# ToughStoneX/Self-Supervised-MVS

Measured on AMD Instinct MI355X. Metric: depth-samples/sec (N=3, 640x512, D=192), higher is better.
Workload: dtype f32

## Files before the change

### self-supervised-mvs_amd/_lib.py

```python
from __future__ import annotations

import contextlib
import ctypes as C
import os

_HERE = os.path.dirname(os.path.abspath(__file__))
LIB_PATH = os.path.join(_HERE, "libmvs_hip.so")

_f = C.c_void_p
_i = C.c_int
_ll = C.c_longlong
_s = C.c_void_p
_fl = C.c_float

class MvsUnetBlock(C.Structure):
    _fields_ = [("transposed", _i), ("stride", _i), ("src", _i), ("skip", _i), ("eps", _fl), ("momentum", _fl),
                ("cin", _i), ("cout", _i), ("d", _i), ("h", _i), ("w", _i)]


class MvsFeatBlock(C.Structure):
    _fields_ = [("cin", _i), ("cout", _i), ("ks", _i), ("stride", _i), ("eps", _fl), ("momentum", _fl), ("w_channels_last", _i),
                ("h", _i), ("w", _i)]


# ... 170 lines not shown
        msg = self._mvs_last_error().decode("utf-8", "replace")
        if rc in (-1, -2, -4):
            raise ValueError("%s failed (%d): %s" % (name, rc, msg))
        raise RuntimeError("%s failed (%d): %s" % (name, rc, msg))

    def raw(self, name: str, *args):
        return getattr(self, "_" + name)(*args)

    def launch_trace(self):
        buf = C.create_string_buffer(4096)
        self._mvs_launch_trace(buf, len(buf))
        return [s for s in buf.value.decode().split(",") if s]

    def get_tuning(self, key: str) -> int:
        v = _i()
        self.call("mvs_get_tuning", key.encode(), C.byref(v))
        return v.value

    @contextlib.contextmanager
    def tuning(self, **knobs):
        old = []
        try:
            for key, val in knobs.items():
                old.append((key, self.get_tuning(key)))
                self.call("mvs_set_tuning", key.encode(), int(val))
            yield self
        finally:
            for key, val in reversed(old):
                self.call("mvs_set_tuning", key.encode(), val)


_INSTANCE = None

DEFAULT_TUNING = {"k8": 7, "xcd": 1, "side_pre": 1, "conv_pers": 1, "conv_pers_min": 1024, "conv_pers_nw": 8, "wgrad_pers": 1, "conv_small": 1, "tr2pw": 1, "sweep_bwd": 0, "wgrad_small": 0, "wgrad_groups": 768, "wgrad8_groups": 192, "wgrad8_gs": 2, "wgrad8_nch": 2, "cout1_h4": 1, "wgrad2d_batch": 2048, "sweep_fwd": 3}


def get() -> MvsLib:
    global _INSTANCE
    if _INSTANCE is None:
        _INSTANCE = MvsLib()
        for item in filter(None, os.environ.get("MVS_TUNING", "").split(",")):
            key, _, val = item.partition("=")
            DEFAULT_TUNING[key.strip()] = int(val)
            _INSTANCE.call("mvs_set_tuning", key.strip().encode(), int(val))
    return _INSTANCE


class KernelTimer:

    def __init__(self, only=None, names=None):
        self.only = only
        self.names = names
        self.events = {}

    def wants(self, name, tag):
        return self.only is None or name in self.only or tag in self.only

    def add(self, name, tag, ev0, ev1):
        self.events.setdefault((name, tag), []).append((ev0, ev1))

    _REG_NAMES = frozenset(("mvs_conv3d_fwd", "mvs_convT3d_fwd", "mvs_conv3d_dgrad", "mvs_convT3d_dgrad", "mvs_conv3d_wgrad", "mvs_convT3d_wgrad",
                            "mvs_bn_relu_fwd_slots", "mvs_bn_relu_bwd_slots", "mvs_bn_bwd_reduce_slots", "mvs_conv3d_pack_weights_batch"))

    def allows_c_entry(self, lib, blocks):
        if self.names is None:
            return False
        hit = self.names & self._REG_NAMES
# ... 57 lines not shown
```

### self-supervised-mvs_amd/csrc/conv3d.hip

```cpp
#include "mvs_rt.h"
#include "conv_map.h"

#include "conv_args.h"

__device__ __forceinline__ void conv_pack_weights_item(const float* __restrict__ w, float* __restrict__ wp, int geom, int CC,
                                                       int Cin, int Cout, int NB, int layout, int flip, int idx) {
    const int j = idx & 3, lane = (idx >> 2) & 63;
    const int nb = (idx >> 8) % NB, kk = (idx >> 8) / NB;
    const int co = nb * 16 + (lane & 15);
    int ks, chunk = 0, cls = 0;
    if (geom == GEOM_TR2_PW) {
        int k0 = 0;
        for (cls = 0; cls < 4; ++cls) {
            int n = tr2p_ntaps(cls) * CC / 16;
            if (kk < k0 + n) break;
            k0 += n;
        }
        ks = kk - k0;
        const int kf = 16 * ks + 4 * (lane >> 4) + j;
        const int tp = kf / CC, cip = kf % CC, n = lane & 15, pw = n >> 3, cop = n & 7;
        int dd, dh, dw, kd, kh;
        tr2p_tap(cls, tp, dd, dh, dw, kd, kh);
        int kw = tr2p_kw(pw, dw);
        float v = 0.f;
// ... 64 lines not shown
template <int NIT, class Map>
__device__ __forceinline__ void stage_load(float4 (&v)[NIT], int (&off)[NIT], int tid, int nitems, Map map) {
#pragma unroll
    for (int k = 0; k < NIT; ++k) {
        const int i = tid + 256 * k;
        off[k] = -1;
        v[k] = make_float4(0.f, 0.f, 0.f, 0.f);
        if (i < nitems) {
            const float* src = nullptr;
            map(i, src, off[k]);
            if (src) v[k] = *reinterpret_cast<const float4*>(src);
        }
    }
}
template <int NIT>
__device__ __forceinline__ void stage_store(float* __restrict__ lds, const float4 (&v)[NIT], const int (&off)[NIT]) {
#pragma unroll
    for (int k = 0; k < NIT; ++k)
        if (off[k] >= 0) *reinterpret_cast<float4*>(lds + off[k]) = v[k];
}
template <int NITEMS, class Map>
__device__ __forceinline__ void stage_batched(float* __restrict__ lds, int tid, Map map) {
    constexpr int NIT = (NITEMS + 255) / 256;
    constexpr int BATCH = NIT < 12 ? NIT : 12;
#pragma unroll
    for (int k0 = 0; k0 < NIT; k0 += BATCH) {
        float4 v[BATCH];
        int off[BATCH];
        stage_load<BATCH>(v, off, tid, NITEMS - 256 * k0, [&](int i, const float*& src, int& o) { map(i + 256 * k0, src, o); });
        stage_store<BATCH>(lds, v, off);
    }
}

template <int GEOM, int CC, int NB, int SIDE>
__global__ __launch_bounds__(256) void conv_igemm_kernel(ConvArgs a) {
    using G = ConvGeom<GEOM>;
    constexpr int CCP = CC + 4;
    constexpr int NR = G::RD * G::RH * G::RW;
    constexpr int MB = G::MB;
    constexpr int CQ = CC / 4;
    __shared__ __attribute__((aligned(16))) float tile[NR * CCP];
    __shared__ int tapoff[32];
    __shared__ float red[4 * NB * 16 * 2];

    const int tid = threadIdx.x, lane = tid & 63, wave = tid >> 6;
    const int g = lane >> 4, l15 = lane & 15;
    const int nb0 = blockIdx.y * NB;

    int t = blockIdx.x;
    const int tw = t % a.ntw; t /= a.ntw;
    const int th = t % a.nth; t /= a.nth;
    const int td = t % a.ntd; t /= a.ntd;
    const int b = t;
    const int qd0 = td * G::TQD, qh0 = th * G::TQH, qw0 = tw * G::TQW;

    if (tid < 32) {
        int off = 0;
        if (G::PW) {
            if (tid < 18) {
                int cls = 0, k0 = 0;
                for (; cls < 4; ++cls) {
                    int n = tr2p_ntaps(cls);
                    if (tid < k0 + n) break;
                    k0 += n;
                }
                int dd, dh, dw, kd, kh;
                tr2p_tap(cls, tid - k0, dd, dh, dw, kd, kh);
                off = ((dd * G::RH + dh) * G::RW + dw) * CCP;
            }
        } else if (G::BASE == GEOM_TR2) {
            if (tid < 27) {
                int cls = 0, k0 = 0;
                for (; cls < 8; ++cls) {
                    int n = tr2_ntaps(cls);
                    if (tid < k0 + n) break;
                    k0 += n;
                }
                int dd, dh, dw, kd, kh, kw;
                tr2_tap(cls, tid - k0, dd, dh, dw, kd, kh, kw);
                off = ((dd * G::RH + dh) * G::RW + dw) * CCP;
            }
        } else if (tid < 27) {
            off = (((tid / 9) * G::RH + (tid / 3) % 3) * G::RW + tid % 3) * CCP;
        }
        tapoff[tid] = off;
    }

    int baseA[MB];
#pragma unroll
    for (int mb = 0; mb < MB; ++mb) {
        const int f = wave * MB + mb;
        const int qd_l = f / G::TQH, qh_l = f % G::TQH;
        baseA[mb] = (((qd_l * G::IS) * G::RH + qh_l * G::IS) * G::RW + l15 * G::IS) * CCP;
    }

    f32x4 acc[MB][NB];
    float st1[NB], st2[NB];
    float bmu[NB], bis[NB], bsc[NB], bsh[NB];
#pragma unroll
    for (int nb = 0; nb < NB; ++nb) {
        st1[nb] = 0.f; st2[nb] = 0.f;
        bmu[nb] = bis[nb] = bsc[nb] = bsh[nb] = 0.f;
        if (SIDE && a.bn_raw) {
            const int co = G::PW ? (l15 & 7) : (nb0 + nb) * 16 + l15;
            if (co < a.Cout) { bmu[nb] = a.bn_stats[co]; bis[nb] = a.bn_stats[a.Cout + co]; bsc[nb] = a.bn_stats[2 * a.Cout + co]; bsh[nb] = a.bn_stats[3 * a.Cout + co]; }
        }
    }

    const int nchunks = G::BASE == GEOM_TR2 ? 1 : a.Cin / CC;
    const int KSF = ksteps_for(27, CC);

    constexpr int EG = (MB * NB * 8 <= 64) ? MB : 1;
    constexpr bool SIDE_PRE = SIDE == 2 && NB == 1 && EG == MB;
    auto pd_of = [&](int cls) { return G::PW ? (cls >> 1) & 1 : (cls >> 2) & 1; };
    auto ph_of = [&](int cls) { return G::PW ? cls & 1 : (cls >> 1) & 1; };
    auto pw_of = [&](int cls) { return G::PW ? (l15 >> 3) : cls & 1; };
    auto load_side = [&](int cls, int mb0, float (&sk)[EG][4][NB], float (&rwv)[EG][4][NB]) {
#pragma unroll
        for (int e = 0; e < EG; ++e) {
            const int f = wave * MB + mb0 + e;
            const int qd = qd0 + f / G::TQH, qh = qh0 + f % G::TQH;
            const int od = qd * G::OS + pd_of(cls), oh = qh * G::OS + ph_of(cls);
#pragma unroll
            for (int r = 0; r < 4; ++r) {
                const int qw = qw0 + 4 * g + r;
                const int ow = qw * G::OS + pw_of(cls);
                const size_t obase = ((((size_t)b * a.Do + od) * a.Ho + oh) * a.Wo + ow) * a.Cout;
#pragma unroll
                for (int nb = 0; nb < NB; ++nb) {
                    const int co = G::PW ? (l15 & 7) : (nb0 + nb) * 16 + l15;
                    const bool ok = qd < a.QD && qh < a.QH && qw < a.QW && co < a.Cout;
                    sk[e][r][nb] = (ok && a.skip) ? a.skip[obase + co] : 0.f;
                    rwv[e][r][nb] = (ok && a.bn_raw) ? a.bn_raw[obase + co] : 0.f;
                }
            }
        }
    };
    float skp[SIDE_PRE ? MB : 1][4][NB], rwp[SIDE_PRE ? MB : 1][4][NB];

    for (int cls = 0; cls < G::NCLS; ++cls) {
#pragma unroll
        for (int mb = 0; mb < MB; ++mb)
#pragma unroll
            for (int nb = 0; nb < NB; ++nb) acc[mb][nb] = (f32x4){0.f, 0.f, 0.f, 0.f};
        if constexpr (SIDE_PRE) {
            if (a.skip || a.bn_raw) load_side(cls, 0, skp, rwp);
        }

        for (int chunk = 0; chunk < nchunks; ++chunk) {
            if (cls == 0) {
                __syncthreads();
                stage_batched<NR * CQ>(tile, tid, [&](int i, const float*& src, int& o) {
                    const int vox = i / CQ, cq = i % CQ;
                    const int rw = vox % G::RW, rh = (vox / G::RW) % G::RH, rd = vox / (G::RW * G::RH);
                    const int id = qd0 * G::IS + rd - G::PAD, ih = qh0 * G::IS + rh - G::PAD,
                              iw = qw0 * G::IS + rw - G::PAD;
                    o = vox * CCP + 4 * cq;
                    if (id >= 0 && id < a.Di && ih >= 0 && ih < a.Hi && iw >= 0 && iw < a.Wi)
                        src = a.x + ((((size_t)b * a.Di + id) * a.Hi + ih) * a.Wi + iw) * a.Cin + chunk * CC + 4 * cq;
                });
                __syncthreads();
            }
            int KS, kk0, tapbase;
            if (G::PW) {
                KS = tr2p_ntaps(cls) * CC / 16;
                tapbase = tr2p_tap_prefix(cls);
                kk0 = tapbase * CC / 16;
            } else if (G::BASE == GEOM_TR2) {
                KS = tr2_ntaps(cls) * CC / 16;
                tapbase = tr2_tap_prefix(cls);
                kk0 = tapbase * CC / 16;
            } else {
                KS = KSF;
                tapbase = 0;
                kk0 = chunk * KSF;
            }
            constexpr int PD = G::BASE == GEOM_TR2 ? 1 : (NB == 1 ? 4 : 2);
            float4 bq[PD][NB], af[MB];
            auto load_b = [&](int ks, float4 (&dst)[NB]) {
                const int kc = ks < KS ? ks : KS - 1;
#pragma unroll
                for (int nb = 0; nb < NB; ++nb)
                    dst[nb] = *reinterpret_cast<const float4*>(a.wp + (((size_t)(kk0 + kc) * a.nb_total + nb0 + nb) * 64 + lane) * 4);
            };
            auto load_a = [&](int ks, float4 (&dst)[MB]) {
                const int kc = ks < KS ? ks : KS - 1;
                const int kflat = 16 * kc + 4 * g;
                const int aoff = tapoff[tapbase + kflat / CC] + kflat % CC;
#pragma unroll
                for (int mb = 0; mb < MB; ++mb) dst[mb] = *reinterpret_cast<const float4*>(&tile[baseA[mb] + aoff]);
            };
#pragma unroll
            for (int u = 0; u < PD; ++u) load_b(u, bq[u]);
            load_a(0, af);
            for (int ks0 = 0; ks0 < KS; ks0 += PD) {
#pragma unroll
                for (int u = 0; u < PD; ++u) {
                    const int ks = ks0 + u;
                    if (ks < KS) {
                        float4 an[MB];
                        load_a(ks + 1, an);
#pragma unroll
                        for (int mb = 0; mb < MB; ++mb)
#pragma unroll
                            for (int nb = 0; nb < NB; ++nb) {
                                acc[mb][nb] = MVS_MFMA_16x16x4(af[mb].x, bq[u][nb].x, acc[mb][nb]);
                                acc[mb][nb] = MVS_MFMA_16x16x4(af[mb].y, bq[u][nb].y, acc[mb][nb]);
                                acc[mb][nb] = MVS_MFMA_16x16x4(af[mb].z, bq[u][nb].z, acc[mb][nb]);
                                acc[mb][nb] = MVS_MFMA_16x16x4(af[mb].w, bq[u][nb].w, acc[mb][nb]);
                            }
                        load_b(ks + PD, bq[u]);
#pragma unroll
                        for (int mb = 0; mb < MB; ++mb) af[mb] = an[mb];
                    }
                }
            }
        }

#pragma unroll
        for (int mb0 = 0; mb0 < MB; mb0 += EG) {
            float sk[EG][4][NB], rwv[EG][4][NB];
            if (SIDE && !SIDE_PRE && (a.skip || a.bn_raw)) load_side(cls, mb0, sk, rwv);
#pragma unroll
            for (int e = 0; e < EG; ++e) {
                const int mb = mb0 + e;
                const int f = wave * MB + mb;
                const int qd = qd0 + f / G::TQH, qh = qh0 + f % G::TQH;
                if (qd >= a.QD || qh >= a.QH) continue;
                const int od = qd * G::OS + pd_of(cls), oh = qh * G::OS + ph_of(cls);
#pragma unroll
                for (int r = 0; r < 4; ++r) {
                    const int qw = qw0 + 4 * g + r;
                    if (qw >= a.QW) continue;
                    const int ow = qw * G::OS + pw_of(cls);
                    const size_t obase = ((((size_t)b * a.Do + od) * a.Ho + oh) * a.Wo + ow) * a.Cout;
#pragma unroll
                    for (int nb = 0; nb < NB; ++nb) {
                        const int co = G::PW ? (l15 & 7) : (nb0 + nb) * 16 + l15;
                        if (co >= a.Cout) continue;
                        float v = acc[mb][nb][r];
                        float sv1 = v, sv2 = v * v;
                        if (a.scale) v = v * a.scale[co] + a.shift[co];
                        else if (a.shift) v = v + a.shift[co];
                        if (a.relu) v = fmaxf(v, 0.f);
                        if (SIDE && a.skip) v += SIDE_PRE ? skp[SIDE_PRE ? mb : 0][r][nb] : sk[e][r][nb];
                        if (SIDE && a.bn_raw) {
                            const float rw = SIDE_PRE ? rwp[SIDE_PRE ? mb : 0][r][nb] : rwv[e][r][nb];
                            sv1 = (rw * bsc[nb] + bsh[nb] > 0.f) ? v : 0.f;
                            sv2 = sv1 * ((rw - bmu[nb]) * bis[nb]);
                        }
                        st1[nb] += sv1;
                        st2[nb] += sv2;
                        a.y[obase + co] = v;
                    }
                }
            }
        }
    }

    if (a.slots) {
#pragma unroll
        for (int nb = 0; nb < NB; ++nb) {
            float s1 = st1[nb], s2 = st2[nb];
            s1 += __shfl_xor(s1, 16); s1 += __shfl_xor(s1, 32);
            s2 += __shfl_xor(s2, 16); s2 += __shfl_xor(s2, 32);
            if (G::PW) { s1 += __shfl_xor(s1, 8); s2 += __shfl_xor(s2, 8); }
            if (lane < 16) {
                red[((wave * NB + nb) * 16 + lane) * 2 + 0] = s1;
// ... 919 lines not shown
    }
    red[slice][el] = (s0 + s1) + (s2 + s3);
    __syncthreads();
    if (slice == 0 && e < n) {
        float t = 0.f;
#pragma unroll
        for (int k = 0; k < 16; ++k) t += red[k][el];
        const int cg = e % CG, cx = (e / CG) % CX, tap = e / (CG * CX);
        gw[((size_t)cg * CX + cx) * 27 + tap] = t;
    }
}

static int pick_cc(int geom, int cin) {
    if (geom == GEOM_TR2) return cin;
    if (geom == GEOM_S2) return 8;
    return (cin % 16 == 0) ? 16 : 8;
}

static int pick_cc_k(int geom, int kgeom, int cin) {
    if (g_tune.cc_wide) {
        if (kgeom == GEOM_S1_SMALL && (cin == 32 || cin == 64)) return cin;
        if (kgeom == GEOM_S2_SMALL && (cin == 16 || cin == 32)) return cin;
    }
    return pick_cc(geom, cin);
}

static size_t packed_floats(int geom, int cin, int cout) {
    const int cc = pick_cc(geom, cin);
    int nb = mvs_cdiv(cout, 16);
    if (nb == 3) nb = 4;
    return (size_t)total_ksteps(geom, cin, cc) * nb * 256;
}

template <int GEOM>
static const char* igemm_label() {
    return GEOM == GEOM_S1 ? "conv_igemm s1" : GEOM == GEOM_S2 ? "conv_igemm s2" : GEOM == GEOM_TR2 ? "conv_igemm tr2" :
           GEOM == GEOM_S1_SMALL ? "conv_igemm s1_small" : GEOM == GEOM_S2_SMALL ? "conv_igemm s2_small" :
           GEOM == GEOM_TR2_SMALL ? "conv_igemm tr2_small" : GEOM == GEOM_TR2_PW ? "conv_igemm tr2_pw" : "conv_igemm";
}

template <int GEOM, int CC>
static int launch_igemm_nb(const ConvArgs& a, int NB, int nblocks, hipStream_t st) {
    dim3 grid(nblocks, a.nb_total / NB), block(256);
    if (a.skip || a.bn_raw) {
        switch (NB) {
            case 1:
                if (g_tune.side_pre) MVS_LAUNCH((conv_igemm_kernel<GEOM, CC, 1, 2>), grid, block, 0, st, a);
                else MVS_LAUNCH((conv_igemm_kernel<GEOM, CC, 1, 1>), grid, block, 0, st, a);
                break;
            case 2: MVS_LAUNCH((conv_igemm_kernel<GEOM, CC, 2, 1>), grid, block, 0, st, a); break;
            case 4: MVS_LAUNCH((conv_igemm_kernel<GEOM, CC, 4, 1>), grid, block, 0, st, a); break;
            default: mvs_set_error("conv igemm: Cout tile count %d unsupported", NB); return MVS_ERR_UNSUPPORTED;
        }
        return mvs_check_launch(igemm_label<GEOM>());
    }
    switch (NB) {
        case 1: MVS_LAUNCH((conv_igemm_kernel<GEOM, CC, 1, 0>), grid, block, 0, st, a); break;
        case 2: MVS_LAUNCH((conv_igemm_kernel<GEOM, CC, 2, 0>), grid, block, 0, st, a); break;
        case 4: MVS_LAUNCH((conv_igemm_kernel<GEOM, CC, 4, 0>), grid, block, 0, st, a); break;
        default: mvs_set_error("conv igemm: Cout tile count %d unsupported", NB); return MVS_ERR_UNSUPPORTED;
    }
    return mvs_check_launch(igemm_label<GEOM>());
}

static void igemm_tiling(int geom, int B, int QD, int QH, int QW, int cout, int& kgeom, int& NB, int& nblocks) {
    const int nb_total = mvs_cdiv(cout, 16) == 3 ? 4 : mvs_cdiv(cout, 16);
    nblocks = B * mvs_cdiv(QD, geom_tqd(geom)) * mvs_cdiv(QH, geom_tqh(geom)) * mvs_cdiv(QW, 16);
    NB = nb_total;
    if (g_tune.conv_split && nblocks < 512 && NB > 1) NB = 1;
    kgeom = geom;
    const long thr = (long)g_tune.conv_small_wgs * (geom == GEOM_S2 ? 24 : (geom == GEOM_S1 ? 3 : 1));
    if (g_tune.conv_small == 2 || (g_tune.conv_small == 1 && (long)nblocks * (nb_total / NB) < thr)) {
        kgeom = geom + GEOM_S1_SMALL;
        nblocks = B * mvs_cdiv(QD, geom_tqd(kgeom)) * mvs_cdiv(QH, geom_tqh(kgeom)) * mvs_cdiv(QW, 16);
    }
}

struct Epilogue {
    const float* scale; const float* shift; const float* skip; int relu;
    double* slots; int nslots;
    const float* bn_raw; const float* bn_stats;
};

struct IgemmPlan {
    int geom, wlayout, flip, B, Di, Hi, Wi, cin, cout;
    bool cin1;
};
enum { MVS_OP_CONV_FWD = 0, MVS_OP_CONV_DGRAD = 1, MVS_OP_CONV_WGRAD = 2,
       MVS_OP_CONVT_FWD = 3, MVS_OP_CONVT_DGRAD = 4, MVS_OP_CONVT_WGRAD = 5 };

static int check_stride(int stride, int D, int H, int W, const char* what) {
    MVS_REQUIRE(stride == 1 || stride == 2, MVS_ERR_UNSUPPORTED, "%s: stride must be 1 or 2, got %d", what, stride);
    MVS_REQUIRE(D > 0 && H > 0 && W > 0, MVS_ERR_SHAPE, "%s: bad spatial shape %dx%dx%d", what, D, H, W);
    return MVS_OK;
}

static int plan_for(int op, int B, int D, int H, int W, int Cin, int Cout, int stride, IgemmPlan& p, const char* what) {
    int rc = check_stride(stride, D, H, W, what);
    if (rc) return rc;
    MVS_REQUIRE(B > 0 && (long long)B * D * H * W * (stride == 2 ? 8 : 1) < (1LL << 31), MVS_ERR_SHAPE,
                "%s: %d x %d x %d x %d voxels do not fit the kernels' 32-bit voxel indices", what, B, D, H, W);
    p = {};
    p.B = B; p.cin1 = false;
    switch (op) {
        case MVS_OP_CONV_FWD:
            p.geom = stride == 2 ? GEOM_S2 : GEOM_S1; p.wlayout = WL_OIK; p.flip = 0;
            p.Di = D; p.Hi = H; p.Wi = W; p.cin = Cin; p.cout = Cout;
// ... 20 lines not shown
            else { p.geom = GEOM_S2; p.Di = 2 * D; p.Hi = 2 * H; p.Wi = 2 * W; }
            return MVS_OK;
        default:
            mvs_set_error("%s: op %d has no weight image", what, op);
            return MVS_ERR_UNSUPPORTED;
    }
}

static void plan_grid(const IgemmPlan& p, int& QD, int& QH, int& QW) {
    if (p.geom == GEOM_S2) { QD = (p.Di - 1) / 2 + 1; QH = (p.Hi - 1) / 2 + 1; QW = (p.Wi - 1) / 2 + 1; }
    else { QD = p.Di; QH = p.Hi; QW = p.Wi; }
}
static bool plan_is_c8(const IgemmPlan& p, const Epilogue* ep) {
    return (g_tune.k8 & 3) && p.geom == GEOM_S1 && p.cout == 8 && (p.cin == 8 || p.cin == 16 || p.cin == 32) && !(ep && ep->bn_raw);
}
static bool plan_is_cout1(const IgemmPlan& p, const Epilogue* ep) {
    return p.geom == GEOM_S1 && p.cout == 1 && p.wlayout == WL_OIK && !p.flip && (p.cin == 8 || p.cin == 16) &&
           !(ep && (ep->slots || ep->bn_raw));
}

static int plan_pack(const IgemmPlan& p, const float* w, float* ws, PackItem& it) {
    it = {};
    it.w = w; it.wp = ws; it.kind = -1;
    if (p.cin1) {
        MVS_REQUIRE(p.cout == 8 || p.cout == 16, MVS_ERR_UNSUPPORTED, "conv3d_dgrad(Cout=1): Cin must be 8 or 16, got %d", p.cout);
        it.kind = 1; it.Cout = p.cout; it.total = 27 * p.cout;
        return MVS_OK;
    }
    MVS_REQUIRE(p.cin == 8 || p.cin == 16 || p.cin == 32 || p.cin == 64, MVS_ERR_UNSUPPORTED,
                "conv igemm: input channels must be 8/16/32/64, got %d", p.cin);
    MVS_REQUIRE(p.cout >= 1 && p.cout <= 64, MVS_ERR_UNSUPPORTED, "conv igemm: output channels must be <= 64, got %d", p.cout);
    MVS_REQUIRE(!(p.geom == GEOM_TR2 && p.cin < 16), MVS_ERR_UNSUPPORTED, "transposed stride-2 conv needs >= 16 input channels");
    int QD, QH, QW, kgeom, NB, nblocks;
    plan_grid(p, QD, QH, QW);
    igemm_tiling(p.geom, p.B, QD, QH, QW, p.cout, kgeom, NB, nblocks);
    const int cc = pick_cc_k(p.geom, kgeom, p.cin);
    const int nb_total = mvs_cdiv(p.cout, 16) == 3 ? 4 : mvs_cdiv(p.cout, 16);
    const int pgeom = (kgeom == GEOM_TR2 && cc == 16 && p.cout == 8 && g_tune.tr2pw) ? GEOM_TR2_PW : p.geom;
    it.kind = 0; it.geom = pgeom; it.CC = cc; it.Cin = p.cin; it.Cout = p.cout; it.NB = nb_total; it.layout = p.wlayout; it.flip = p.flip;
    it.total = (int)((size_t)total_ksteps(pgeom, p.cin, cc) * nb_total * 256);
    return MVS_OK;
}

static int launch_pack(const PackItem* items, int n, hipStream_t st) {
    for (int i0 = 0; i0 < n; i0 += MVS_PACK_BATCH_MAX) {
        PackBatch pb = {};
        int m = 0, maxtotal = 0;
        for (int i = i0; i < n && m < MVS_PACK_BATCH_MAX; ++i) {
            if (items[i].kind < 0) continue;
            pb.it[m++] = items[i];
            if (items[i].total > maxtotal) maxtotal = items[i].total;
        }
        if (m == 0) continue;
        MVS_LAUNCH(conv_pack_batch_kernel, dim3(mvs_cdiv(maxtotal, 256), m), dim3(256), 0, st, pb);
    }
    return mvs_check_launch("conv_pack_weights");
}

static int run_igemm(const IgemmPlan& p, const float* in, const float* wsrc, float* out, float* ws, const Epilogue& ep,
                     int ws_packed, hipStream_t st) {
    MVS_REQUIRE(in && wsrc && out && ws, MVS_ERR_NULL, "conv: null pointer argument");
    MVS_REQUIRE(!ep.slots || (ep.nslots >= 1 && ep.nslots <= 256 && (ep.nslots & (ep.nslots - 1)) == 0), MVS_ERR_SHAPE,
                "conv: statistic slot count must be a power of two <= 256, got %d", ep.nslots);
    MVS_REQUIRE(!ep.bn_raw || (ep.bn_stats && ep.slots), MVS_ERR_NULL, "conv: bn_raw needs bn_stats and slots");
    const int geom = p.geom, B = p.B, cin = p.cin, cout = p.cout;
    ConvArgs a = {};
    a.x = in; a.y = out; a.B = B; a.Di = p.Di; a.Hi = p.Hi; a.Wi = p.Wi; a.Cin = cin; a.Cout = cout;
    a.scale = ep.scale; a.shift = ep.shift; a.skip = ep.skip; a.relu = ep.relu;
    a.slots = ep.slots; a.nslots = ep.nslots; a.bn_raw = ep.bn_raw; a.bn_stats = ep.bn_stats;
    plan_grid(p, a.QD, a.QH, a.QW);
    if (geom == GEOM_S1) { a.Do = p.Di; a.Ho = p.Hi; a.Wo = p.Wi; }
    else if (geom == GEOM_S2) { a.Do = a.QD; a.Ho = a.QH; a.Wo = a.QW; }
    else { a.Do = 2 * p.Di; a.Ho = 2 * p.Hi; a.Wo = 2 * p.Wi; }
    a.ntd = mvs_cdiv(a.QD, geom_tqd(geom)); a.nth = mvs_cdiv(a.QH, geom_tqh(geom)); a.ntw = mvs_cdiv(a.QW, 16);
    if ((g_tune.conv0_x3 & 1) && conv_x3_serves(geom, a)) return run_conv_x3(a, wsrc, p.wlayout, p.flip, st);
    if ((g_tune.conv0_x3 & 2) && conv_x3_fwd_serves(geom, a)) return run_conv_x3_fwd(a, wsrc, p.wlayout, p.flip, ws, st);
    if (plan_is_c8(p, &ep)) {
        const int ntl = B * a.ntd * a.nth * a.ntw;
        const int nbc = ntl < 512 ? ntl : 512;
        if (cin == 32) MVS_LAUNCH((conv_c8_fwd_bc_kernel<16, 2>), dim3(nbc), dim3(256), 0, st, a, wsrc, p.wlayout, p.flip, g_tune.xcd);
        else if (cin == 16) MVS_LAUNCH((conv_c8_fwd_bc_kernel<16, 1>), dim3(nbc), dim3(256), 0, st, a, wsrc, p.wlayout, p.flip, g_tune.xcd);
        else MVS_LAUNCH((conv_c8_fwd_bc_kernel<8, 1>), dim3(nbc), dim3(256), 0, st, a, wsrc, p.wlayout, p.flip, g_tune.xcd);
        return mvs_check_launch("conv_c8_fwd_bc");
    }
    int nblocks = B * a.ntd * a.nth * a.ntw;
    if (plan_is_cout1(p, &ep)) {
        if (cin == 8 && g_tune.cout1_h4) {
            a.ntd = mvs_cdiv(a.QD, CO1_TD); a.nth = mvs_cdiv(a.QH, CO1_TH); a.ntw = mvs_cdiv(a.QW, CO1_TW);
            MVS_LAUNCH(conv_cout1_h4_kernel, dim3(B * a.ntd * a.nth * a.ntw), dim3(256), 0, st, a, wsrc);
        } else if (cin == 8) MVS_LAUNCH((conv_cout1_kernel<8>), dim3(nblocks), dim3(256), 0, st, a, wsrc);
        else MVS_LAUNCH((conv_cout1_kernel<16>), dim3(nblocks), dim3(256), 0, st, a, wsrc);
        return mvs_check_launch(cin == 8 ? (g_tune.cout1_h4 ? "conv_cout1 h4" : "conv_cout1 cin=8") : "conv_cout1 cin=16");
    }
    int NB, kgeom;
    a.nb_total = mvs_cdiv(cout, 16) == 3 ? 4 : mvs_cdiv(cout, 16);
    igemm_tiling(geom, B, a.QD, a.QH, a.QW, cout, kgeom, NB, nblocks);
    const int cc = pick_cc_k(geom, kgeom, cin);
    a.ntd = mvs_cdiv(a.QD, geom_tqd(kgeom)); a.nth = mvs_cdiv(a.QH, geom_tqh(kgeom));
    if (!ws_packed) {
        PackItem it;
        int rc = plan_pack(p, wsrc, ws, it);
        if (rc) return rc;
        rc = launch_pack(&it, 1, st);
        if (rc) return rc;
    } else {
        MVS_REQUIRE(cin == 8 || cin == 16 || cin == 32 || cin == 64, MVS_ERR_UNSUPPORTED, "conv igemm: input channels must be 8/16/32/64, got %d", cin);
        MVS_REQUIRE(cout >= 1 && cout <= 64, MVS_ERR_UNSUPPORTED, "conv igemm: output channels must be <= 64, got %d", cout);
        MVS_REQUIRE(!(geom == GEOM_TR2 && cin < 16), MVS_ERR_UNSUPPORTED, "transposed stride-2 conv needs >= 16 input channels");
    }
    a.wp = ws;
    if (g_tune.conv_pers && conv_pers_serves(geom, cin, cout) && (long)nblocks * (a.nb_total / NB) >= g_tune.conv_pers_min) {
        a.ntd = mvs_cdiv(a.QD, geom_tqd(geom)); a.nth = mvs_cdiv(a.QH, geom_tqh(geom));
        return run_conv_pers(geom, a, st);
    }
    if ((g_tune.conv_pers & 1) && kgeom == GEOM_TR2 && cc == 16 && cout == 8 && g_tune.tr2pw && conv_pers_serves(GEOM_TR2_PW, cin, cout) &&
        nblocks >= g_tune.conv_pers_min)
        return run_conv_pers(GEOM_TR2_PW, a, st);
    if (kgeom == GEOM_S1) return cc == 16 ? launch_igemm_nb<GEOM_S1, 16>(a, NB, nblocks, st)
                                          : launch_igemm_nb<GEOM_S1, 8>(a, NB, nblocks, st);
    if (kgeom == GEOM_S2) return launch_igemm_nb<GEOM_S2, 8>(a, NB, nblocks, st);
    if (kgeom == GEOM_S1_SMALL) {
        if (cc == 64) return launch_igemm_nb<GEOM_S1_SMALL, 64>(a, NB, nblocks, st);
        if (cc == 32) return launch_igemm_nb<GEOM_S1_SMALL, 32>(a, NB, nblocks, st);
        return cc == 16 ? launch_igemm_nb<GEOM_S1_SMALL, 16>(a, NB, nblocks, st) : launch_igemm_nb<GEOM_S1_SMALL, 8>(a, NB, nblocks, st);
    }
    if (kgeom == GEOM_S2_SMALL) {
        if (cc == 32) return launch_igemm_nb<GEOM_S2_SMALL, 32>(a, NB, nblocks, st);
        if (cc == 16) return launch_igemm_nb<GEOM_S2_SMALL, 16>(a, NB, nblocks, st);
        return launch_igemm_nb<GEOM_S2_SMALL, 8>(a, NB, nblocks, st);
    }
    if (kgeom == GEOM_TR2_SMALL) {
        if (cc == 16) return launch_igemm_nb<GEOM_TR2_SMALL, 16>(a, NB, nblocks, st);
        if (cc == 32) return launch_igemm_nb<GEOM_TR2_SMALL, 32>(a, NB, nblocks, st);
        return launch_igemm_nb<GEOM_TR2_SMALL, 64>(a, NB, nblocks, st);
    }
    if (cc == 16 && cout == 8 && g_tune.tr2pw) return launch_igemm_nb<GEOM_TR2_PW, 16>(a, NB, nblocks, st);
    if (cc == 16) return launch_igemm_nb<GEOM_TR2, 16>(a, NB, nblocks, st);
    if (cc == 32) return launch_igemm_nb<GEOM_TR2, 32>(a, NB, nblocks, st);
    return launch_igemm_nb<GEOM_TR2, 64>(a, NB, nblocks, st);
}

static int run_cin1(const IgemmPlan& p, const float* gy, const float* w, float* gx, float* ws, const Epilogue& ep, int ws_packed,
                    hipStream_t st) {
    MVS_REQUIRE(gy && w && gx && ws, MVS_ERR_NULL, "conv3d_dgrad: null pointer argument");
    MVS_REQUIRE(!ep.skip, MVS_ERR_UNSUPPORTED, "conv3d_dgrad: the Cout = 1 input gradient takes no summand");
    MVS_REQUIRE(!ep.bn_raw || (ep.bn_stats && ep.slots), MVS_ERR_NULL, "conv3d_dgrad: bn_raw needs bn_stats and slots");
    MVS_REQUIRE(!ep.slots || (ep.bn_raw && ep.nslots >= 1 && ep.nslots <= 256 && (ep.nslots & (ep.nslots - 1)) == 0), MVS_ERR_SHAPE,
                "conv3d_dgrad: bad statistic slots");
    const int C = p.cout;
    if (!ws_packed) {
        PackItem it;
        int rc = plan_pack(p, w, ws, it);
        if (rc) return rc;
        rc = launch_pack(&it, 1, st);
        if (rc) return rc;
    } else {
        MVS_REQUIRE(C == 8 || C == 16, MVS_ERR_UNSUPPORTED, "conv3d_dgrad(Cout=1): Cin must be 8 or 16, got %d", C);
    }
    const size_t total = (size_t)p.B * p.Di * p.Hi * p.Wi;
    const int vpt = (g_tune.cin1_vpt == 5 || (g_tune.cin1_vpt == 4 && total >= (size_t)1 << 20)) ? 4 : 1;
    dim3 grid((unsigned)((total + 256 * vpt - 1) / (256 * vpt)));
    if (C == 8 && vpt == 4) MVS_LAUNCH((conv_cin1_kernel<8, 4>), grid, dim3(256), 0, st, gy, (const float*)ws, gx, p.B, p.Di, p.Hi, p.Wi, ep.bn_raw, ep.bn_stats, ep.slots, ep.nslots);
// ... 206 lines not shown
```

### self-supervised-mvs_amd/csrc/tuning.h

```cpp
#pragma once

#define MVS_KNOBS(X) \
     \
    X(nt,               0,    0, 1,       "forward: non-temporal stores of the variance volume") \
    X(tile_w,           0,    0, 256,     "cached forward: pixel-tile width, 0 = the default tile") \
    X(dslab,            0,    0, 1 << 20, "forward: planes per workgroup, 0 = auto") \
    X(sweep_fwd,        3,    0, 4,       "forward: 0 taps through L1 every plane, 1 LDS-staged windows, 2 register-cached taps (4 ch/thread), 3 (8 ch/thread), 4 (16 ch/thread, <= 2 source views)") \
    X(sweep_bwd,        0,    0, 1,       "backward: 0 per-wave windows (<= 4 source views), 1 view-pair kernel with LDS atomics (what > 4 source views run)") \
    X(bwd_dslab,        0,    0, 1 << 20, "per-wave-window backward: planes per workgroup, 0 = auto") \
    X(bwd_nowin,        0,    0, 1,       "(tests) 1 = no LDS windows, every flush through global atomics") \
    X(bwd_cpt,          4,    4, 8,       "accepted and ignored (the 8-channels-per-thread backward was measured slower and removed)") \
    X(bwd_pf,           0,    0, 2,       "backward: 1 = block lookahead for 1-2 source views, 2 = ONE wave per SIMD for 3-4 source views") \
    X(bwd_gd,           2,    0, 2,       "backward: 2 = upstream gradient requested two planes ahead at 2 waves/SIMD (1-2 source views), 0 = rotating set at 3 waves/SIMD") \
    X(bwd_gd34,         0,    0, 1,       "backward: 3-4 source views with the upstream gradient requested two planes ahead (as 1-2 views run), 2 waves/SIMD") \
    X(fwd_pt,           0,    0, 1,       "cached forward with the per-wave projection table (plane_sweep_variance_fwd_pt_kernel): measured and rejected") \
    X(bwd_gpf,          0,    0, 1,       "per-wave-window backward requests the next planes' upstream gradient: 0 top of the group, 1 after the plane's gathers") \
    X(fwd_dl,           2,    0, 2,       "forward: 0 the round-1 loop, 1 LDS-staged per-plane depths, 2 + all views' re-gathers in flight before the first sample") \
    X(sweep_xcd,        0,    0, 1,       "XCD-compact workgroup order of the cached forward and the per-wave-window backward") \
     \
    X(conv_split,       1,    0, 1,       "0 keeps all Cout tiles in one workgroup") \
    X(conv_small,       1,    0, 2,       "quarter-size workgroup tiles for under-filled launches (0 never, 1 auto, 2 always)") \
    X(conv_small_wgs,   384,  0, 1 << 20, "... below this many workgroups (~1.5 per CU)") \
    X(tr2pw,            1,    0, 1,       "transposed stride-2 conv with Cout == 8 as W-parity-merged GEMMs (GEOM_TR2_PW)") \
    X(cc_wide,          0,    0, 1,       "quarter-tile kernels of the deep levels with all input channels as one chunk: measured and rejected") \
    X(cin1_vpt,         1,    1, 5,       "voxels per thread of the Cout == 1 layer's input gradient (4 = four from 1 M voxels on, 5 = always four): measured and rejected") \
    X(k8,               7,    0, 15,      "bit mask: 1|2 = Cout == 8 stride-1 layers run the 4x4x1 MFMA forward with the weights as the broadcast operand (0: generic kernel), +4 = weight gradient with g as the broadcast operand") \
    X(cout1_d4,         2,    0, 3,       "bit 1: the Cout = 1 layer of the bf16 inference path with four outputs per thread") \
    X(cout1_h4,         1,    0, 1,       "the 8 -> 1 layer with four outputs per thread (conv_cout1_h4_kernel); 0: one output per thread") \
    X(bf16_dp,          1,    0, 1,       "conv0 of the bf16 path (32 -> 8) with two output depth slices per MFMA (GEOM_S1_DP)") \
    X(xcd,              1,    0, 1,       "XCD-aware tile order in the broadcast-operand forward and the Cout == 8 weight gradient") \
    X(side_pre,         1,    0, 1,       "one-Cout-tile kernels with epilogue side inputs (skip / bn_raw) request them before the k-loop (1) or at the top of the epilogue (0)") \
    X(conv_pers,        1,    0, 1,       "one-chunk layers (16 -> <= 16, 8 -> 32 stride 1; 8 -> <= 16 stride 2) run the persistent kernels of conv3d_pers.hip") \
    X(conv_pers_min,    1024, 0, 1 << 30, "... when the one-tile kernel would launch at least this many workgroups (a persistent grid needs several tiles per workgroup)") \
    X(conv_pers_groups, 0,    0, 4096,    "workgroups of a persistent launch, 0 = what fits the GPU (tests: a few workgroups walk many tiles)") \
    X(conv_pers_nw,     8,    4, 8,       "waves per workgroup of conv_pers_kernel") \
    X(wgrad_pers,       1,    0, 1,       "one-chunk weight gradients run conv3d_pers.hip, from conv_pers_min tiles on") \
    X(wgrad_small,      0,    0, 3,       "quarter-size tiles in the generic weight-gradient kernel: 1 = 8-channel / stride-2 layers with many tiles, 2 = every layer with many tiles, 3 = always (tests)") \
    X(wgrad_groups,     768,  1, 768,     "persistent workgroups of the generic weight-gradient kernels") \
    X(wgrad8_groups,    192,  1, 512,     "... of the CG == 8 kernel (conv0)") \
    X(wgrad8_gs,        2,    0, 2,       "conv0's weight gradient in the output-gradient-shifted form on the 16x16x4 MFMA (conv_c8_wgrad_gs_kernel): 1 eight waves per workgroup, 2 sixteen; 0: conv_c8_wgrad_kernel (4x4x1 MFMA, X shifted)") \
    X(wgrad8_nch,       2,    1, 2,       "2 = the CG == 8 weight gradient stages both 16-channel chunks of a 32-channel X in one workgroup") \
    X(conv0_x3,         0,    0, 3,       "split-bf16 products (conv3d_x3.hip, opt-in): bit 0 = conv0's input gradient, bit 1 = conv0's forward") \
     \
    X(conv2d_pp,        1,    0, 1,       "3x3 stride-1 layers with <= 8 output channels as pixel-pair GEMMs (conv2d_igemm_kernel<.., PP>)") \
    X(conv2d_s2_mfma,   2,    0, 2,       "stride-2 input gradient: 2 ONE four-class MFMA pass with compacted taps, 1 four parity-class passes, 0 direct VALU form") \
    X(wgrad2d_groups,   256,  0, 1 << 20, "persistent workgroups of the weight gradient (used: 1 .. 1024; 256 = one per CU)") \
    X(wgrad2d_batch,    2048, 1, 4096,    "workgroups of the batched weight gradient (both launches together), shared out by work") \
     \
    X(c2w_tile,         0,    0, 2,       "0 = t128x64 when its launch has at least c2w_big_min workgroups, else t64x64; 1 = always t64x64; 2 = always t128x64") \
    X(c2w_big_min,      512,  0, 1 << 30, "... workgroups (two per CU)") \
    X(c2w_splitk,       0,    0, 8,       "K ranges of a layer: 0 = doubled (<= 8) while a t64x64 launch has fewer than c2w_split_min workgroups, 1 = never split, 2..8 = this many") \
    X(c2w_split_min,    512,  0, 1 << 30, "... workgroups (two per CU)") \
    X(c2w_bf_split_min, 2048, 0, 1 << 30, "c2w_split_min of the bf16 arms (arith = bf16): eight workgroups per CU")

struct MvsTuning {
#define MVS_KNOB_FIELD(key, def, lo, hi, doc) int key;
// ... 5 lines not shown
```

Before: 214.3.

## Add H-major quarter tiles and next-chunk halo prefetch to igemm conv

Adds an H-major variant of the quarter-size implicit-GEMM conv tiles: the 16-wide M axis runs along H instead of W. It is chosen automatically when that orientation gives fewer tiles, which cuts partial-tile waste on odd shapes. It also adds register prefetch of the next channel chunk's halo, issued under the current k-loop, so the global load overlaps the MFMA work instead of stalling between chunks. Both come at the cost of more template instantiations and extra registers for the prefetch buffers, which may lower occupancy.

After: 216.1, median of 6. Within noise of the previous version (+0.8%).

```diff
diff --git a/self-supervised-mvs_amd/_lib.py b/self-supervised-mvs_amd/_lib.py
--- a/self-supervised-mvs_amd/_lib.py
+++ b/self-supervised-mvs_amd/_lib.py
@@ -226,7 +226,7 @@
 
 _INSTANCE = None
 
-DEFAULT_TUNING = {"k8": 7, "xcd": 1, "side_pre": 1, "conv_pers": 1, "conv_pers_min": 1024, "conv_pers_nw": 8, "wgrad_pers": 1, "conv_small": 1, "tr2pw": 1, "sweep_bwd": 0, "wgrad_small": 0, "wgrad_groups": 768, "wgrad8_groups": 192, "wgrad8_gs": 2, "wgrad8_nch": 2, "cout1_h4": 1, "wgrad2d_batch": 2048, "sweep_fwd": 3}
+DEFAULT_TUNING = {"k8": 7, "xcd": 1, "side_pre": 1, "conv_pers": 1, "conv_pers_min": 1024, "conv_pers_nw": 8, "wgrad_pers": 1, "conv_small": 1, "conv_hmajor": 1, "conv_chunk_pf": 1, "tr2pw": 1, "sweep_bwd": 0, "wgrad_small": 0, "wgrad_groups": 768, "wgrad8_groups": 192, "wgrad8_gs": 2, "wgrad8_nch": 2, "cout1_h4": 1, "wgrad2d_batch": 2048, "sweep_fwd": 3}
 
 
 def get() -> MvsLib:
diff --git a/self-supervised-mvs_amd/csrc/conv3d.hip b/self-supervised-mvs_amd/csrc/conv3d.hip
--- a/self-supervised-mvs_amd/csrc/conv3d.hip
+++ b/self-supervised-mvs_amd/csrc/conv3d.hip
@@ -120,9 +120,11 @@
     }
 }
 
-template <int GEOM, int CC, int NB, int SIDE>
+template <int GEOM, int CC, int NB, int SIDE, int HM = 0, int PF = 0>
 __global__ __launch_bounds__(256) void conv_igemm_kernel(ConvArgs a) {
     using G = ConvGeom<GEOM>;
+    static_assert(!HM || (GEOM >= GEOM_S1_SMALL && GEOM <= GEOM_TR2_SMALL), "H-major tiles: quarter-size geometries only");
+    static_assert(!PF || G::BASE != GEOM_TR2, "the transposed geometry has one chunk");
     constexpr int CCP = CC + 4;
     constexpr int NR = G::RD * G::RH * G::RW;
     constexpr int MB = G::MB;
@@ -140,7 +142,7 @@
     const int th = t % a.nth; t /= a.nth;
     const int td = t % a.ntd; t /= a.ntd;
     const int b = t;
-    const int qd0 = td * G::TQD, qh0 = th * G::TQH, qw0 = tw * G::TQW;
+    const int qd0 = td * G::TQD, qh0 = th * (HM ? 16 : G::TQH), qw0 = tw * (HM ? G::TQH : G::TQW);
 
     if (tid < 32) {
         int off = 0;
@@ -166,10 +168,11 @@
                 }
                 int dd, dh, dw, kd, kh, kw;
                 tr2_tap(cls, tid - k0, dd, dh, dw, kd, kh, kw);
-                off = ((dd * G::RH + dh) * G::RW + dw) * CCP;
+                off = HM ? ((dd * G::RH + dw) * G::RW + dh) * CCP : ((dd * G::RH + dh) * G::RW + dw) * CCP;
             }
         } else if (tid < 27) {
-            off = (((tid / 9) * G::RH + (tid / 3) % 3) * G::RW + tid % 3) * CCP;
+            off = HM ? (((tid / 9) * G::RH + tid % 3) * G::RW + (tid / 3) % 3) * CCP
+                     : (((tid / 9) * G::RH + (tid / 3) % 3) * G::RW + tid % 3) * CCP;
         }
         tapoff[tid] = off;
     }
@@ -207,17 +210,17 @@
 #pragma unroll
         for (int e = 0; e < EG; ++e) {
             const int f = wave * MB + mb0 + e;
-            const int qd = qd0 + f / G::TQH, qh = qh0 + f % G::TQH;
-            const int od = qd * G::OS + pd_of(cls), oh = qh * G::OS + ph_of(cls);
+            const int qd = qd0 + f / G::TQH, qr = (HM ? qw0 : qh0) + f % G::TQH;
+            const int od = qd * G::OS + pd_of(cls), orow = qr * G::OS + (HM ? pw_of(cls) : ph_of(cls));
 #pragma unroll
             for (int r = 0; r < 4; ++r) {
-                const int qw = qw0 + 4 * g + r;
-                const int ow = qw * G::OS + pw_of(cls);
-                const size_t obase = ((((size_t)b * a.Do + od) * a.Ho + oh) * a.Wo + ow) * a.Cout;
+                const int qm = (HM ? qh0 : qw0) + 4 * g + r;
+                const int om = qm * G::OS + (HM ? ph_of(cls) : pw_of(cls));
+                const size_t obase = ((((size_t)b * a.Do + od) * a.Ho + (HM ? om : orow)) * a.Wo + (HM ? orow : om)) * a.Cout;
 #pragma unroll
                 for (int nb = 0; nb < NB; ++nb) {
                     const int co = G::PW ? (l15 & 7) : (nb0 + nb) * 16 + l15;
-                    const bool ok = qd < a.QD && qh < a.QH && qw < a.QW && co < a.Cout;
+                    const bool ok = qd < a.QD && qr < (HM ? a.QW : a.QH) && qm < (HM ? a.QH : a.QW) && co < a.Cout;
                     sk[e][r][nb] = (ok && a.skip) ? a.skip[obase + co] : 0.f;
                     rwv[e][r][nb] = (ok && a.bn_raw) ? a.bn_raw[obase + co] : 0.f;
                 }
@@ -226,6 +229,27 @@
     };
     float skp[SIDE_PRE ? MB : 1][4][NB], rwp[SIDE_PRE ? MB : 1][4][NB];
 
+    auto halo_map = [&](int chunk) {
+        return [&a, b, qd0, qh0, qw0, chunk](int i, const float*& src, int& o) {
+            const int vox = i / CQ, cq = i % CQ;
+            int rd, rh, rw;
+            if (HM) {
+                rw = vox % G::RH; rh = (vox / G::RH) % G::RW; rd = vox / (G::RW * G::RH);
+                o = ((rd * G::RH + rw) * G::RW + rh) * CCP + 4 * cq;
+            } else {
+                rw = vox % G::RW; rh = (vox / G::RW) % G::RH; rd = vox / (G::RW * G::RH);
+                o = vox * CCP + 4 * cq;
+            }
+            const int id = qd0 * G::IS + rd - G::PAD, ih = qh0 * G::IS + rh - G::PAD,
+                      iw = qw0 * G::IS + rw - G::PAD;
+            if (id >= 0 && id < a.Di && ih >= 0 && ih < a.Hi && iw >= 0 && iw < a.Wi)
+                src = a.x + ((((size_t)b * a.Di + id) * a.Hi + ih) * a.Wi + iw) * a.Cin + chunk * CC + 4 * cq;
+        };
+    };
+    constexpr int PFN = PF ? (NR * CQ + 255) / 256 : 1;
+    float4 pfv[PFN];
+    int pfo[PFN];
+
     for (int cls = 0; cls < G::NCLS; ++cls) {
 #pragma unroll
         for (int mb = 0; mb < MB; ++mb)
@@ -237,17 +261,28 @@
 
         for (int chunk = 0; chunk < nchunks; ++chunk) {
             if (cls == 0) {
-                __syncthreads();
-                stage_batched<NR * CQ>(tile, tid, [&](int i, const float*& src, int& o) {
-                    const int vox = i / CQ, cq = i % CQ;
-                    const int rw = vox % G::RW, rh = (vox / G::RW) % G::RH, rd = vox / (G::RW * G::RH);
-                    const int id = qd0 * G::IS + rd - G::PAD, ih = qh0 * G::IS + rh - G::PAD,
-                              iw = qw0 * G::IS + rw - G::PAD;
-                    o = vox * CCP + 4 * cq;
-                    if (id >= 0 && id < a.Di && ih >= 0 && ih < a.Hi && iw >= 0 && iw < a.Wi)
-                        src = a.x + ((((size_t)b * a.Di + id) * a.Hi + ih) * a.Wi + iw) * a.Cin + chunk * CC + 4 * cq;
-                });
-                __syncthreads();
+                if constexpr (PF) {
+                    if (chunk == 0) stage_load<PFN>(pfv, pfo, tid, NR * CQ, halo_map(0));
+                    __syncthreads();
+                    stage_store<PFN>(tile, pfv, pfo);
+                    __syncthreads();
+                } else if constexpr (HM) {
+                    __syncthreads();
+                    stage_batched<NR * CQ>(tile, tid, halo_map(chunk));
+                    __syncthreads();
+                } else {
+                    __syncthreads();
+                    stage_batched<NR * CQ>(tile, tid, [&](int i, const float*& src, int& o) {
+                        const int vox = i / CQ, cq = i % CQ;
+                        const int rw = vox % G::RW, rh = (vox / G::RW) % G::RH, rd = vox / (G::RW * G::RH);
+                        const int id = qd0 * G::IS + rd - G::PAD, ih = qh0 * G::IS + rh - G::PAD,
+                                  iw = qw0 * G::IS + rw - G::PAD;
+                        o = vox * CCP + 4 * cq;
+                        if (id >= 0 && id < a.Di && ih >= 0 && ih < a.Hi && iw >= 0 && iw < a.Wi)
+                            src = a.x + ((((size_t)b * a.Di + id) * a.Hi + ih) * a.Wi + iw) * a.Cin + chunk * CC + 4 * cq;
+                    });
+                    __syncthreads();
+                }
             }
             int KS, kk0, tapbase;
             if (G::PW) {
@@ -281,6 +316,9 @@
 #pragma unroll
             for (int u = 0; u < PD; ++u) load_b(u, bq[u]);
             load_a(0, af);
+            if constexpr (PF) {
+                if (chunk + 1 < nchunks) stage_load<PFN>(pfv, pfo, tid, NR * CQ, halo_map(chunk + 1));
+            }
             for (int ks0 = 0; ks0 < KS; ks0 += PD) {
 #pragma unroll
                 for (int u = 0; u < PD; ++u) {
@@ -313,15 +351,15 @@
             for (int e = 0; e < EG; ++e) {
                 const int mb = mb0 + e;
                 const int f = wave * MB + mb;
-                const int qd = qd0 + f / G::TQH, qh = qh0 + f % G::TQH;
-                if (qd >= a.QD || qh >= a.QH) continue;
-                const int od = qd * G::OS + pd_of(cls), oh = qh * G::OS + ph_of(cls);
+                const int qd = qd0 + f / G::TQH, qr = (HM ? qw0 : qh0) + f % G::TQH;
+                if (qd >= a.QD || qr >= (HM ? a.QW : a.QH)) continue;
+                const int od = qd * G::OS + pd_of(cls), orow = qr * G::OS + (HM ? pw_of(cls) : ph_of(cls));
 #pragma unroll
                 for (int r = 0; r < 4; ++r) {
-                    const int qw = qw0 + 4 * g + r;
-                    if (qw >= a.QW) continue;
-                    const int ow = qw * G::OS + pw_of(cls);
-                    const size_t obase = ((((size_t)b * a.Do + od) * a.Ho + oh) * a.Wo + ow) * a.Cout;
+                    const int qm = (HM ? qh0 : qw0) + 4 * g + r;
+                    if (qm >= (HM ? a.QH : a.QW)) continue;
+                    const int om = qm * G::OS + (HM ? ph_of(cls) : pw_of(cls));
+                    const size_t obase = ((((size_t)b * a.Do + od) * a.Ho + (HM ? om : orow)) * a.Wo + (HM ? orow : om)) * a.Cout;
 #pragma unroll
                     for (int nb = 0; nb < NB; ++nb) {
                         const int co = G::PW ? (l15 & 7) : (nb0 + nb) * 16 + l15;
@@ -1307,47 +1345,59 @@
     return (size_t)total_ksteps(geom, cin, cc) * nb * 256;
 }
 
-template <int GEOM>
+template <int GEOM, int HM = 0>
 static const char* igemm_label() {
+    if (HM) return GEOM == GEOM_S1_SMALL ? "conv_igemm s1_small hm" : GEOM == GEOM_S2_SMALL ? "conv_igemm s2_small hm" : "conv_igemm tr2_small hm";
     return GEOM == GEOM_S1 ? "conv_igemm s1" : GEOM == GEOM_S2 ? "conv_igemm s2" : GEOM == GEOM_TR2 ? "conv_igemm tr2" :
            GEOM == GEOM_S1_SMALL ? "conv_igemm s1_small" : GEOM == GEOM_S2_SMALL ? "conv_igemm s2_small" :
            GEOM == GEOM_TR2_SMALL ? "conv_igemm tr2_small" : GEOM == GEOM_TR2_PW ? "conv_igemm tr2_pw" : "conv_igemm";
 }
 
-template <int GEOM, int CC>
+template <int GEOM, int CC, int HM = 0, int PF = 0>
 static int launch_igemm_nb(const ConvArgs& a, int NB, int nblocks, hipStream_t st) {
     dim3 grid(nblocks, a.nb_total / NB), block(256);
     if (a.skip || a.bn_raw) {
         switch (NB) {
             case 1:
-                if (g_tune.side_pre) MVS_LAUNCH((conv_igemm_kernel<GEOM, CC, 1, 2>), grid, block, 0, st, a);
-                else MVS_LAUNCH((conv_igemm_kernel<GEOM, CC, 1, 1>), grid, block, 0, st, a);
+                if (g_tune.side_pre) MVS_LAUNCH((conv_igemm_kernel<GEOM, CC, 1, 2, HM, PF>), grid, block, 0, st, a);
+                else MVS_LAUNCH((conv_igemm_kernel<GEOM, CC, 1, 1, HM, PF>), grid, block, 0, st, a);
                 break;
-            case 2: MVS_LAUNCH((conv_igemm_kernel<GEOM, CC, 2, 1>), grid, block, 0, st, a); break;
-            case 4: MVS_LAUNCH((conv_igemm_kernel<GEOM, CC, 4, 1>), grid, block, 0, st, a); break;
+            case 2: MVS_LAUNCH((conv_igemm_kernel<GEOM, CC, 2, 1, HM, PF>), grid, block, 0, st, a); break;
+            case 4: MVS_LAUNCH((conv_igemm_kernel<GEOM, CC, 4, 1, HM, PF>), grid, block, 0, st, a); break;
             default: mvs_set_error("conv igemm: Cout tile count %d unsupported", NB); return MVS_ERR_UNSUPPORTED;
         }
-        return mvs_check_launch(igemm_label<GEOM>());
+        return mvs_check_launch(igemm_label<GEOM, HM>());
     }
     switch (NB) {
-        case 1: MVS_LAUNCH((conv_igemm_kernel<GEOM, CC, 1, 0>), grid, block, 0, st, a); break;
-        case 2: MVS_LAUNCH((conv_igemm_kernel<GEOM, CC, 2, 0>), grid, block, 0, st, a); break;
-        case 4: MVS_LAUNCH((conv_igemm_kernel<GEOM, CC, 4, 0>), grid, block, 0, st, a); break;
+        case 1: MVS_LAUNCH((conv_igemm_kernel<GEOM, CC, 1, 0, HM, PF>), grid, block, 0, st, a); break;
+        case 2: MVS_LAUNCH((conv_igemm_kernel<GEOM, CC, 2, 0, HM, PF>), grid, block, 0, st, a); break;
+        case 4: MVS_LAUNCH((conv_igemm_kernel<GEOM, CC, 4, 0, HM, PF>), grid, block, 0, st, a); break;
         default: mvs_set_error("conv igemm: Cout tile count %d unsupported", NB); return MVS_ERR_UNSUPPORTED;
     }
-    return mvs_check_launch(igemm_label<GEOM>());
-}
-
-static void igemm_tiling(int geom, int B, int QD, int QH, int QW, int cout, int& kgeom, int& NB, int& nblocks) {
+    return mvs_check_launch(igemm_label<GEOM, HM>());
+}
+
+static bool hmajor_compiled(int kgeom, int cc) {
+    return kgeom == GEOM_S1_SMALL ? cc == 16 : kgeom == GEOM_S2_SMALL ? cc == 8 : kgeom == GEOM_TR2_SMALL;
+}
+static const bool kHmajorAuto[3] = {true, true, true};
+static const bool kChunkPf[3] = {true, true, false};
+
+static void igemm_tiling(int geom, int B, int QD, int QH, int QW, int cin, int cout, int& kgeom, int& NB, int& nblocks, bool& hm) {
     const int nb_total = mvs_cdiv(cout, 16) == 3 ? 4 : mvs_cdiv(cout, 16);
     nblocks = B * mvs_cdiv(QD, geom_tqd(geom)) * mvs_cdiv(QH, geom_tqh(geom)) * mvs_cdiv(QW, 16);
     NB = nb_total;
     if (g_tune.conv_split && nblocks < 512 && NB > 1) NB = 1;
     kgeom = geom;
+    hm = false;
     const long thr = (long)g_tune.conv_small_wgs * (geom == GEOM_S2 ? 24 : (geom == GEOM_S1 ? 3 : 1));
     if (g_tune.conv_small == 2 || (g_tune.conv_small == 1 && (long)nblocks * (nb_total / NB) < thr)) {
         kgeom = geom + GEOM_S1_SMALL;
-        nblocks = B * mvs_cdiv(QD, geom_tqd(kgeom)) * mvs_cdiv(QH, geom_tqh(kgeom)) * mvs_cdiv(QW, 16);
+        const int tqh = geom_tqh(kgeom);
+        const int wmajor = mvs_cdiv(QH, tqh) * mvs_cdiv(QW, 16), hmajor = mvs_cdiv(QH, 16) * mvs_cdiv(QW, tqh);
+        hm = hmajor_compiled(kgeom, pick_cc_k(geom, kgeom, cin)) &&
+             (g_tune.conv_hmajor == 2 || (g_tune.conv_hmajor == 1 && kHmajorAuto[geom] && hmajor < wmajor));
+        nblocks = B * mvs_cdiv(QD, geom_tqd(kgeom)) * wmajor;
     }
 }
 
@@ -1434,8 +1484,9 @@
     MVS_REQUIRE(p.cout >= 1 && p.cout <= 64, MVS_ERR_UNSUPPORTED, "conv igemm: output channels must be <= 64, got %d", p.cout);
     MVS_REQUIRE(!(p.geom == GEOM_TR2 && p.cin < 16), MVS_ERR_UNSUPPORTED, "transposed stride-2 conv needs >= 16 input channels");
     int QD, QH, QW, kgeom, NB, nblocks;
+    bool hm;
     plan_grid(p, QD, QH, QW);
-    igemm_tiling(p.geom, p.B, QD, QH, QW, p.cout, kgeom, NB, nblocks);
+    igemm_tiling(p.geom, p.B, QD, QH, QW, p.cin, p.cout, kgeom, NB, nblocks, hm);
     const int cc = pick_cc_k(p.geom, kgeom, p.cin);
     const int nb_total = mvs_cdiv(p.cout, 16) == 3 ? 4 : mvs_cdiv(p.cout, 16);
     const int pgeom = (kgeom == GEOM_TR2 && cc == 16 && p.cout == 8 && g_tune.tr2pw) ? GEOM_TR2_PW : p.geom;
@@ -1495,10 +1546,12 @@
         return mvs_check_launch(cin == 8 ? (g_tune.cout1_h4 ? "conv_cout1 h4" : "conv_cout1 cin=8") : "conv_cout1 cin=16");
     }
     int NB, kgeom;
+    bool hm;
     a.nb_total = mvs_cdiv(cout, 16) == 3 ? 4 : mvs_cdiv(cout, 16);
-    igemm_tiling(geom, B, a.QD, a.QH, a.QW, cout, kgeom, NB, nblocks);
+    igemm_tiling(geom, B, a.QD, a.QH, a.QW, cin, cout, kgeom, NB, nblocks, hm);
     const int cc = pick_cc_k(geom, kgeom, cin);
     a.ntd = mvs_cdiv(a.QD, geom_tqd(kgeom)); a.nth = mvs_cdiv(a.QH, geom_tqh(kgeom));
+    const bool pf = g_tune.conv_chunk_pf && cin / cc > 1 && geom != GEOM_TR2 && kChunkPf[geom];
     if (!ws_packed) {
         PackItem it;
         int rc = plan_pack(p, wsrc, ws, it);
@@ -1518,18 +1571,31 @@
     if ((g_tune.conv_pers & 1) && kgeom == GEOM_TR2 && cc == 16 && cout == 8 && g_tune.tr2pw && conv_pers_serves(GEOM_TR2_PW, cin, cout) &&
         nblocks >= g_tune.conv_pers_min)
         return run_conv_pers(GEOM_TR2_PW, a, st);
+    if (hm) {
+        a.nth = mvs_cdiv(a.QH, 16); a.ntw = mvs_cdiv(a.QW, geom_tqh(kgeom));
+        nblocks = B * a.ntd * a.nth * a.ntw;
+    }
     if (kgeom == GEOM_S1) return cc == 16 ? launch_igemm_nb<GEOM_S1, 16>(a, NB, nblocks, st)
                                           : launch_igemm_nb<GEOM_S1, 8>(a, NB, nblocks, st);
     if (kgeom == GEOM_S2) return launch_igemm_nb<GEOM_S2, 8>(a, NB, nblocks, st);
     if (kgeom == GEOM_S1_SMALL) {
         if (cc == 64) return launch_igemm_nb<GEOM_S1_SMALL, 64>(a, NB, nblocks, st);
         if (cc == 32) return launch_igemm_nb<GEOM_S1_SMALL, 32>(a, NB, nblocks, st);
+        if (cc == 16 && hm) return pf ? launch_igemm_nb<GEOM_S1_SMALL, 16, 1, 1>(a, NB, nblocks, st) : launch_igemm_nb<GEOM_S1_SMALL, 16, 1, 0>(a, NB, nblocks, st);
+        if (cc == 16 && pf) return launch_igemm_nb<GEOM_S1_SMALL, 16, 0, 1>(a, NB, nblocks, st);
         return cc == 16 ? launch_igemm_nb<GEOM_S1_SMALL, 16>(a, NB, nblocks, st) : launch_igemm_nb<GEOM_S1_SMALL, 8>(a, NB, nblocks, st);
     }
     if (kgeom == GEOM_S2_SMALL) {
         if (cc == 32) return launch_igemm_nb<GEOM_S2_SMALL, 32>(a, NB, nblocks, st);
         if (cc == 16) return launch_igemm_nb<GEOM_S2_SMALL, 16>(a, NB, nblocks, st);
+        if (hm) return pf ? launch_igemm_nb<GEOM_S2_SMALL, 8, 1, 1>(a, NB, nblocks, st) : launch_igemm_nb<GEOM_S2_SMALL, 8, 1, 0>(a, NB, nblocks, st);
+        if (pf) return launch_igemm_nb<GEOM_S2_SMALL, 8, 0, 1>(a, NB, nblocks, st);
         return launch_igemm_nb<GEOM_S2_SMALL, 8>(a, NB, nblocks, st);
+    }
+    if (kgeom == GEOM_TR2_SMALL && hm) {
+        if (cc == 16) return launch_igemm_nb<GEOM_TR2_SMALL, 16, 1>(a, NB, nblocks, st);
+        if (cc == 32) return launch_igemm_nb<GEOM_TR2_SMALL, 32, 1>(a, NB, nblocks, st);
+        return launch_igemm_nb<GEOM_TR2_SMALL, 64, 1>(a, NB, nblocks, st);
     }
     if (kgeom == GEOM_TR2_SMALL) {
         if (cc == 16) return launch_igemm_nb<GEOM_TR2_SMALL, 16>(a, NB, nblocks, st);
diff --git a/self-supervised-mvs_amd/csrc/tuning.h b/self-supervised-mvs_amd/csrc/tuning.h
--- a/self-supervised-mvs_amd/csrc/tuning.h
+++ b/self-supervised-mvs_amd/csrc/tuning.h
@@ -22,6 +22,8 @@
     X(conv_small,       1,    0, 2,       "quarter-size workgroup tiles for under-filled launches (0 never, 1 auto, 2 always)") \
     X(conv_small_wgs,   384,  0, 1 << 20, "... below this many workgroups (~1.5 per CU)") \
     X(tr2pw,            1,    0, 1,       "transposed stride-2 conv with Cout == 8 as W-parity-merged GEMMs (GEOM_TR2_PW)") \
+    X(conv_hmajor,      1,    0, 2,       "quarter-size tiles with the 16-wide M axis along H instead of W (0 never, 1 auto: when that gives strictly fewer tiles, 2 always: tests)") \
+    X(conv_chunk_pf,    1,    0, 1,       "quarter-size tiles with several channel chunks request the next chunk's halo under the k-loop (0: load, wait, write LDS between the k-loops)") \
     X(cc_wide,          0,    0, 1,       "quarter-tile kernels of the deep levels with all input channels as one chunk: measured and rejected") \
     X(cin1_vpt,         1,    1, 5,       "voxels per thread of the Cout == 1 layer's input gradient (4 = four from 1 M voxels on, 5 = always four): measured and rejected") \
     X(k8,               7,    0, 15,      "bit mask: 1|2 = Cout == 8 stride-1 layers run the 4x4x1 MFMA forward with the weights as the broadcast operand (0: generic kernel), +4 = weight gradient with g as the broadcast operand") \
```
